# huggingface/parler-tts

Hardware: NVIDIA H100
Metric: audio codec tokens/sec (all codebooks) (higher is better)
Workload: dtype bf16

## Files before the change

### parler_tts_b200/csrc/sample_core.cuh

```cuda
#pragma once
#include "common.cuh"
#include "kernels.h"

namespace ptts {

__device__ __forceinline__ uint32_t fkey(float f) {
  uint32_t u = __float_as_uint(f);
  return (u & 0x80000000u) ? ~u : (u | 0x80000000u);
}

__device__ __forceinline__ void philox_round(uint32_t (&c)[4], uint32_t k0, uint32_t k1) {
  const uint32_t hi0 = __umulhi(0xD2511F53u, c[0]), lo0 = 0xD2511F53u * c[0];
  const uint32_t hi1 = __umulhi(0xCD9E8D57u, c[2]), lo1 = 0xCD9E8D57u * c[2];
  c[0] = hi1 ^ c[1] ^ k0; c[1] = lo1; c[2] = hi0 ^ c[3] ^ k1; c[3] = lo0;
}
__device__ __forceinline__ float philox_uniform(uint64_t seed, uint32_t row, uint32_t col) {
  uint32_t c[4] = {row, col, 0x5054u, 0x5453u};
  uint32_t k0 = (uint32_t)seed, k1 = (uint32_t)(seed >> 32);
#pragma unroll
  for (int i = 0; i < 10; i++) { philox_round(c, k0, k1); k0 += 0x9E3779B9u; k1 += 0xBB67AE85u; }
  return (float)(c[0] >> 8) * (1.0f / 16777216.0f);
}


constexpr int SMP_WARPS = 8;
constexpr int SMP_THREADS = SMP_WARPS * 32;

constexpr int SMP_MAX_ROWS = 3;
struct SmpScratch {
  float f[2][SMP_MAX_ROWS][SMP_WARPS];
  int i[2][SMP_MAX_ROWS][SMP_WARPS];
  int z[2][SMP_MAX_ROWS][SMP_WARPS];
};
__device__ __forceinline__ SmpScratch& smp_scratch() {
  __shared__ SmpScratch sc;
  return sc;
}
constexpr int SMP_BAN_WORDS = 9 * SMP_THREADS / 32;
__device__ __forceinline__ uint32_t (&smp_bans())[SMP_MAX_ROWS][SMP_BAN_WORDS] {
  __shared__ uint32_t ban[SMP_MAX_ROWS][SMP_BAN_WORDS];
  return ban;
}

template <int ITEMS, int R, bool EXT = false>
__device__ __forceinline__ void sample_rows_cta(const SampleArgs& p, const ptts_gen_params& g, const int64_t* __restrict__ forced,
                                                int row0, int stride, int n_rows, int cur_len, ptts_sampling_ext x = {},
                                                SampleOut o = {}) {
  static_assert(R >= 1 && R <= SMP_MAX_ROWS, "rows per pass");
  SmpScratch& sc = smp_scratch();
  float (&s_f)[2][SMP_MAX_ROWS][SMP_WARPS] = sc.f;
  int (&s_i)[2][SMP_MAX_ROWS][SMP_WARPS] = sc.i;
  int (&s_z)[2][SMP_MAX_ROWS][SMP_WARPS] = sc.z;
  const int tid = threadIdx.x, lane = tid & 31, warp = tid >> 5;
  int buf = 0;
  auto cta_sum_i = [&](int (&v)[R]) {
#pragma unroll
    for (int r = 0; r < R; r++) {
      const int w = __reduce_add_sync(0xffffffffu, v[r]);
      if (lane == 0) s_i[buf][r][warp] = w;
    }
    __syncthreads();
#pragma unroll
    for (int r = 0; r < R; r++) {
      int a = 0;
#pragma unroll
      for (int w = 0; w < SMP_WARPS; w++) a += s_i[buf][r][w];
      v[r] = a;
    }
    buf ^= 1;
  };
  auto cta_sum_f = [&](float (&v)[R]) {
#pragma unroll
    for (int r = 0; r < R; r++) {
      const float w = warp_sum(v[r]);
      if (lane == 0) s_f[buf][r][warp] = w;
    }
    __syncthreads();
#pragma unroll
    for (int r = 0; r < R; r++) {
      float a = 0.f;
#pragma unroll
      for (int w = 0; w < SMP_WARPS; w++) a += s_f[buf][r][w];
      v[r] = a;
    }
    buf ^= 1;
  };
  auto cta_max_f = [&](float (&v)[R]) {
#pragma unroll
    for (int r = 0; r < R; r++) {
      const float w = warp_max(v[r]);
      if (lane == 0) s_f[buf][r][warp] = w;
    }
    __syncthreads();
#pragma unroll
    for (int r = 0; r < R; r++) {
      float a = s_f[buf][r][0];
#pragma unroll
      for (int w = 1; w < SMP_WARPS; w++) a = fmaxf(a, s_f[buf][r][w]);
      v[r] = a;
    }
    buf ^= 1;
  };

  int row[R];
  bool valid[R];
  float v[R][ITEMS];
#pragma unroll
  for (int r = 0; r < R; r++) {
    row[r] = row0 + r * stride;
    valid[r] = row[r] < n_rows;
#pragma unroll
    for (int j = 0; j < ITEMS; j++) {
      const int i = tid + SMP_THREADS * j;
      v[r][j] = (valid[r] && i < p.V) ? __ldcg(p.logits + (size_t)row[r] * p.V + i) : -INFINITY;
    }
  }
  auto out_row = [&](float* base, int r) -> float* {
    const int step = cur_len - (g.input_len > 1 ? g.input_len : 1);
    if (base == nullptr || !valid[r] || step < o.first_step || step - o.first_step >= o.n_steps) return nullptr;
    return base + (int64_t)(step - o.first_step) * o.step_stride + (int64_t)row[r] * p.V;
  };
  if constexpr (EXT) {
#pragma unroll
    for (int r = 0; r < R; r++) {
      if (float* dst = out_row(o.logits, r)) {
#pragma unroll
        for (int j = 0; j < ITEMS; j++) {
          const int i = tid + SMP_THREADS * j;
          if (i < p.V) __stcs(dst + i, v[r][j]);
        }
      }
    }
  }
  int t_unf = 0, t_es = 0;
  if (tid < R && row0 + tid * stride < n_rows) { t_unf = p.unfinished[row0 + tid * stride]; t_es = p.eos_seen[row0 + tid * stride]; }
  const int ngram = EXT ? x.no_repeat_ngram_size : 0;
  const bool bans = EXT && ngram > 0 && cur_len + 1 >= ngram;
  if constexpr (EXT) {
    if (bans) {
      uint32_t (&ban)[SMP_MAX_ROWS][SMP_BAN_WORDS] = smp_bans();
#pragma unroll
      for (int r = 0; r < R; r++)
        for (int w = tid; w < SMP_BAN_WORDS; w += SMP_THREADS) ban[r][w] = 0u;
      __syncthreads();
#pragma unroll
      for (int r = 0; r < R; r++) {
        if (!valid[r]) continue;
        const int64_t* h = p.raw_ids + (size_t)row[r] * p.raw_ld;
        const int64_t* tail = h + cur_len - ngram + 1;
        for (int i = tid; i <= cur_len - ngram; i += SMP_THREADS) {
          bool match = true;
          for (int q = 0; q < ngram - 1 && match; q++) match = h[i + q] == tail[q];
          const int64_t t = h[i + ngram - 1];
          if (match && t >= 0 && t < p.V) atomicOr(&ban[r][t >> 5], 1u << (t & 31));
        }
      }
      __syncthreads();
    }
  }
#pragma unroll
  for (int r = 0; r < R; r++) {
    const int b = row[r] / p.K, k = row[r] - b * p.K;
    bool mask_eos = false;
    if (cur_len - (g.input_len > 1 ? g.input_len : 1) < g.min_new_tokens) mask_eos = true;
    if (valid[r]) {
      const int par = cur_len & 1;
      int fu = p.first_unf[par * p.B + b];
      const int es = __ldcg(p.eos_seen + fu);
      if (es > 0 && es <= cur_len && fu < b * p.K + p.K - 1) fu++;
      if (k == 0 && tid == 0) p.first_unf[(par ^ 1) * p.B + b] = fu;
      if (row[r] > fu) mask_eos = true;
    }
#pragma unroll
    for (int j = 0; j < ITEMS; j++) {
      const int i = tid + SMP_THREADS * j;
      if (mask_eos && i == p.eos) v[r][j] = -INFINITY;
      if (g.suppress_special && i >= g.codebook_size) v[r][j] = -INFINITY;
      if constexpr (EXT)
        if (bans && ((smp_bans()[r][i >> 5] >> (i & 31)) & 1u)) v[r][j] = -INFINITY;
    }
  }
  int tok[R];
#pragma unroll
  for (int r = 0; r < R; r++) tok[r] = 0;
  if (g.do_sample) {
    if (g.temperature != 1.0f) {
#pragma unroll
      for (int r = 0; r < R; r++)
#pragma unroll
        for (int j = 0; j < ITEMS; j++) v[r][j] = v[r][j] / g.temperature;
    }
    if (g.top_k > 0) {
      const int kk = g.top_k < p.V ? g.top_k : p.V;
      uint32_t key[R][ITEMS];
      uint32_t th[R];
#pragma unroll
      for (int r = 0; r < R; r++) {
        th[r] = 0;
#pragma unroll
        for (int j = 0; j < ITEMS; j++) key[r][j] = (tid + SMP_THREADS * j < p.V) ? fkey(v[r][j]) : 0u;
      }
      for (int bit = 31; bit >= 0; bit--) {
        int cnt[R];
#pragma unroll
        for (int r = 0; r < R; r++) {
          const uint32_t cand = th[r] | (1u << bit);
          cnt[r] = 0;
#pragma unroll
          for (int j = 0; j < ITEMS; j++) cnt[r] += (key[r][j] >= cand) ? 1 : 0;
        }
        cta_sum_i(cnt);
#pragma unroll
        for (int r = 0; r < R; r++)
          if (cnt[r] >= kk) th[r] |= (1u << bit);
      }
#pragma unroll
      for (int r = 0; r < R; r++)
#pragma unroll
        for (int j = 0; j < ITEMS; j++)
          if (fkey(v[r][j]) < th[r]) v[r][j] = -INFINITY;
    }
    float m[R];
#pragma unroll
    for (int r = 0; r < R; r++) {
      m[r] = -INFINITY;
#pragma unroll
      for (int j = 0; j < ITEMS; j++) m[r] = fmaxf(m[r], v[r][j]);
    }
    cta_max_f(m);
    float e[R][ITEMS];
    float s[R];
#pragma unroll
    for (int r = 0; r < R; r++) {
      s[r] = 0.f;
#pragma unroll
      for (int j = 0; j < ITEMS; j++) { e[r][j] = expf(v[r][j] - m[r]); s[r] += e[r][j]; }
    }
    cta_sum_f(s);
    if (g.top_p < 1.0f) {
      uint32_t th[R];
#pragma unroll
      for (int r = 0; r < R; r++) th[r] = 0;
      for (int bit = 31; bit >= 0; bit--) {
        float c[R];
#pragma unroll
        for (int r = 0; r < R; r++) {
          const uint32_t cand = th[r] | (1u << bit);
          c[r] = 0.f;
#pragma unroll
          for (int j = 0; j < ITEMS; j++) c[r] += (fkey(v[r][j]) <= cand) ? e[r][j] : 0.f;
        }
        cta_sum_f(c);
#pragma unroll
        for (int r = 0; r < R; r++)
          if (c[r] <= (1.0f - g.top_p) * s[r]) th[r] |= (1u << bit);
      }
#pragma unroll
      for (int r = 0; r < R; r++) {
        const uint32_t kmax = fkey(m[r]);
        s[r] = 0.f;
#pragma unroll
        for (int j = 0; j < ITEMS; j++) {
          const uint32_t key = fkey(v[r][j]);
          if (key <= th[r] && key != kmax) { v[r][j] = -INFINITY; e[r][j] = 0.f; }
          s[r] += e[r][j];
        }
      }
      cta_sum_f(s);
    }
    if constexpr (EXT) {
      auto drop_where = [&](auto&& remove) {
#pragma unroll
        for (int r = 0; r < R; r++) {
          const float inv = 1.0f / s[r];
          s[r] = 0.f;
#pragma unroll
          for (int j = 0; j < ITEMS; j++) {
            if (remove(r, j, inv)) { v[r][j] = -INFINITY; e[r][j] = 0.f; }
            s[r] += e[r][j];
          }
        }
        cta_sum_f(s);
      };
      auto entropy = [&](float (&ent)[R], float (&lse)[R]) {
#pragma unroll
        for (int r = 0; r < R; r++) {
          lse[r] = m[r] + logf(s[r]);
          ent[r] = 0.f;
#pragma unroll
          for (int j = 0; j < ITEMS; j++)
            if (v[r][j] > -INFINITY) { const float lp = v[r][j] - lse[r]; ent[r] += lp * expf(lp); }
        }
        cta_sum_f(ent);
#pragma unroll
        for (int r = 0; r < R; r++) ent[r] = -ent[r];
      };
      if (x.min_p > 0.f)
        drop_where([&](int r, int j, float inv) { return e[r][j] * inv < x.min_p * inv; });
      if (x.typical_p < 1.0f) {
        float ent[R], lse[R];
        entropy(ent, lse);
        uint32_t key[R][ITEMS], th[R];
#pragma unroll
        for (int r = 0; r < R; r++) {
          th[r] = 0;
#pragma unroll
          for (int j = 0; j < ITEMS; j++) key[r][j] = fkey(v[r][j] > -INFINITY ? fabsf(lse[r] - v[r][j] - ent[r]) : INFINITY);
        }
        for (int bit = 31; bit >= 0; bit--) {
          float c[R];
#pragma unroll
          for (int r = 0; r < R; r++) {
            const uint32_t cand = th[r] | (1u << bit);
            c[r] = 0.f;
#pragma unroll
            for (int j = 0; j < ITEMS; j++) c[r] += (key[r][j] <= cand) ? e[r][j] : 0.f;
          }
          cta_sum_f(c);
#pragma unroll
          for (int r = 0; r < R; r++)
            if (c[r] < x.typical_p * s[r]) th[r] |= (1u << bit);
        }
        drop_where([&](int r, int j, float) { return th[r] != 0xffffffffu && key[r][j] > th[r] + 1u; });
      }
      if (x.epsilon_cutoff > 0.f)
        drop_where([&](int r, int j, float inv) { return e[r][j] * inv < x.epsilon_cutoff && v[r][j] < m[r]; });
      if (x.eta_cutoff > 0.f) {
        float ent[R], lse[R];
        entropy(ent, lse);
        drop_where([&](int r, int j, float inv) {
          return e[r][j] * inv < fminf(x.eta_cutoff, sqrtf(x.eta_cutoff) * expf(-ent[r])) && v[r][j] < m[r];
        });
      }
    }
    float target[R], carry[R];
    int found[R], last_nz[R];
#pragma unroll
    for (int r = 0; r < R; r++) {
      target[r] = philox_uniform(g.seed, (uint32_t)(row[r] + g.row_base), (uint32_t)cur_len) * s[r];
      carry[r] = 0.f; found[r] = -1; last_nz[r] = -1;
    }
#pragma unroll
    for (int j = 0; j < ITEMS; j++) {
      float x[R];
#pragma unroll
      for (int r = 0; r < R; r++) {
        x[r] = e[r][j];
#pragma unroll
        for (int o = 1; o < 32; o <<= 1) {
          const float y = __shfl_up_sync(0xffffffffu, x[r], o);
          if (lane >= o) x[r] += y;
        }
        if (lane == 31) s_f[buf][r][warp] = x[r];
      }
      __syncthreads();
      float tot[R];
#pragma unroll
      for (int r = 0; r < R; r++) {
        float base = carry[r];
        tot[r] = carry[r];
#pragma unroll
        for (int w = 0; w < SMP_WARPS; w++) {
          const float tw = s_f[buf][r][w];
          if (w < warp) base += tw;
          tot[r] += tw;
        }
        const float cum = base + x[r];
        const unsigned hit = __ballot_sync(0xffffffffu, cum > target[r] && e[r][j] > 0.f);
        const unsigned nz = __ballot_sync(0xffffffffu, e[r][j] > 0.f);
        if (lane == 0) {
          s_i[buf][r][warp] = hit ? SMP_THREADS * j + 32 * warp + (__ffs(hit) - 1) : 0x7fffffff;
          s_z[buf][r][warp] = nz ? SMP_THREADS * j + 32 * warp + (31 - __clz(nz)) : -1;
        }
      }
      __syncthreads();
#pragma unroll
      for (int r = 0; r < R; r++) {
        int first = 0x7fffffff, lastz = -1;
#pragma unroll
        for (int w = 0; w < SMP_WARPS; w++) { first = min(first, s_i[buf][r][w]); lastz = max(lastz, s_z[buf][r][w]); }
        if (found[r] < 0 && first != 0x7fffffff) found[r] = first;
        if (lastz >= 0) last_nz[r] = lastz;
        carry[r] = tot[r];
      }
      buf ^= 1;
    }
#pragma unroll
    for (int r = 0; r < R; r++) tok[r] = found[r] >= 0 ? found[r] : last_nz[r];
    if constexpr (EXT) {
#pragma unroll
      for (int r = 0; r < R; r++)
        if (tok[r] < 0) tok[r] = 0;
    }
  } else {
#pragma unroll
    for (int r = 0; r < R; r++) {
      float m = -INFINITY;
      int mi = 0x7fffffff;
#pragma unroll
      for (int j = 0; j < ITEMS; j++) {
        const int i = tid + SMP_THREADS * j;
        if (i < p.V && (v[r][j] > m || (v[r][j] == m && i < mi))) { m = v[r][j]; mi = i; }
      }
#pragma unroll
      for (int o = 16; o > 0; o >>= 1) {
        const float om = __shfl_xor_sync(0xffffffffu, m, o);
        const int oi = __shfl_xor_sync(0xffffffffu, mi, o);
        if (om > m || (om == m && oi < mi)) { m = om; mi = oi; }
      }
      if (lane == 0) { s_f[buf][r][warp] = m; s_i[buf][r][warp] = mi; }
    }
    __syncthreads();
#pragma unroll
    for (int r = 0; r < R; r++) {
      float m = s_f[buf][r][0];
      int mi = s_i[buf][r][0];
#pragma unroll
      for (int w = 1; w < SMP_WARPS; w++) {
        const float om = s_f[buf][r][w];
        const int oi = s_i[buf][r][w];
        if (om > m || (om == m && oi < mi)) { m = om; mi = oi; }
      }
      tok[r] = mi;
    }
    buf ^= 1;
  }
#pragma unroll
  for (int r = 0; r < R; r++) {
    if (!valid[r]) continue;
#pragma unroll
    for (int j = 0; j < ITEMS; j++) {
      const int i = tid + SMP_THREADS * j;
      if (i < p.V) p.scores[(size_t)row[r] * p.V + i] = v[r][j];
    }
    if constexpr (EXT) {
      if (float* dst = out_row(o.scores, r)) {
#pragma unroll
        for (int j = 0; j < ITEMS; j++) {
          const int i = tid + SMP_THREADS * j;
          if (i < p.V) __stcs(dst + i, v[r][j]);
        }
      }
    }
  }
  int my_tok = 0, my_row = 0;
  bool my_valid = false;
#pragma unroll
  for (int r = 0; r < R; r++)
    if (tid == r) { my_tok = tok[r]; my_row = row[r]; my_valid = valid[r]; }
  if (tid < R && my_valid) {
    const int b = my_row / p.K, k = my_row - b * p.K;
    int t = my_tok;
    if (forced != nullptr) t = (int)forced[my_row];
    if (!t_unf) t = p.pad;
    p.raw_ids[(size_t)my_row * p.raw_ld + cur_len] = t;
    if (t == p.eos && t_es == 0) p.eos_seen[my_row] = cur_len + 1;
    const int new_len = cur_len + 1;
    const int done = (t == p.eos) || (new_len >= g.max_length);
    const int still_unfinished = t_unf && !done;
    p.unfinished[my_row] = still_unfinished;
    int nxt = t;
    if (g.max_length >= 2 * p.K - 1) {
      const bool is_bos = cur_len <= k;
      const bool is_pad = (cur_len - k) >= (g.max_length - p.K + 1);
      if (is_bos || is_pad) nxt = (is_bos ? p.bos : 0) + (is_pad ? p.pad : 0);
      else if (g.input_len > 1 && cur_len - g.input_len < k) nxt = (int)p.prefix_cells[(size_t)my_row * (p.K - 1) + (cur_len - g.input_len)];
    }
    p.cur_ids[my_row] = nxt;
    if (still_unfinished) atomicAdd(&p.ctrl->n_unfinished, 1);
  }
  __syncthreads();
}

template <int ITEMS>
__device__ __forceinline__ void sample_row_cta(const SampleArgs& p, const ptts_gen_params& g, const int64_t* __restrict__ forced,
                                               int row, int cur_len) {
  sample_rows_cta<ITEMS, 1>(p, g, forced, row, 0, row + 1, cur_len);
}

template <int ITEMS>
__device__ __forceinline__ void sample_all_rows_cta(const SampleArgs& p, const ptts_gen_params& g, int cta, int n_ctas, int n_rows, int cur_len) {
  if (n_rows <= n_ctas) {
    if (cta < n_rows) sample_rows_cta<ITEMS, 1>(p, g, nullptr, cta, n_ctas, n_rows, cur_len);
  } else {
    for (int row0 = cta; row0 < n_rows; row0 += 3 * n_ctas) sample_rows_cta<ITEMS, 3>(p, g, nullptr, row0, n_ctas, n_rows, cur_len);
  }
}

}
```

### parler_tts_b200/csrc/step2.cu

```cuda
#include "attn_core.cuh"
#include "common.cuh"
#include "kernels.h"
#include "ln_stats.cuh"
#include "sample_core.cuh"
#include "ptx.cuh"
#include "step.h"
#include "step_common.cuh"
#include <type_traits>

namespace ptts {
namespace cl {

constexpr int C = 2;
constexpr int V = 8;
constexpr int THREADS = 256;
constexpr int ROWS = 32;
constexpr int HROWS = 8;
constexpr int ATT_SMEM = attn_decode_smem_per_warp<bf16>();
constexpr int PROF_STRIDE = 16;
constexpr int QMAX = 6;
constexpr int OFF_STATS = 256, OFF_PART = 512, OFF_RES = 2560, OFF_CVEC = 3584;
constexpr int HDR = 5632;
constexpr int WB_BYTES = 65536;
constexpr int R_OFF = HDR + 2 * WB_BYTES;
// ... 121 lines not shown
  const int dgrp = warp & 1, e4 = warp >> 1;

  uint64_t* abar = reinterpret_cast<uint64_t*>(smem);
  uint64_t* wbar = abar + 1;
  uint64_t* xbar = abar + 3;
  uint64_t* attbars = reinterpret_cast<uint64_t*>(smem + 128);
  float* stats = reinterpret_cast<float*>(smem + OFF_STATS);
  float* part = reinterpret_cast<float*>(smem + OFF_PART);
  float* res_s = reinterpret_cast<float*>(smem + OFF_RES);
  float* cvec = reinterpret_cast<float*>(smem + OFF_CVEC);
  unsigned char* Rg = smem + R_OFF;
  const uint32_t peer_xbar = mapa(smem_u32(xbar), (uint32_t)peer);
  uint32_t par_a = 0, par_w = 0, par_x = 0, att_parity = 0;

  if (tid == 0) {
    mbar_init<1>(abar); mbar_init<1>(&wbar[0]); mbar_init<1>(&wbar[1]); mbar_init<1>(xbar);
    asm volatile("fence.mbarrier_init.release.cluster;" ::: "memory");
  }
  attention_decode_init_warp(attbars + 2 * warp, lane);
  cluster_arrive(); cluster_wait();
  unsigned* const bar_ctr = p.bar + (gen & 1u);
  unsigned bar_target = 0u;
  if (cta == 0 && tid == 0) p.bar[(gen + 1u) & 1u] = 0u;

  const char* blob = p.blob;
  long long* const prof0 = (p.prof != nullptr && cta == 0) ? p.prof : nullptr;
  long long* prof = prof0;
  prof_mark(prof, 0);

  auto issue_weight_job = [&](int j) {
    const char* src; uint32_t bytes;
    if (!weight_job(p, j, cta, rank, src, bytes)) return;
    mbar_expect_tx(&wbar[j & 1], bytes);
    bulk_g2s_evict_first(smem + HDR + (j & 1) * WB_BYTES, src, bytes, &wbar[j & 1]);
  };
  __shared__ int s_next_active;
  const int n_steps = (p.do_sample_phase && p.n_steps > 1 && prof0 == nullptr) ? p.n_steps : 1;
  int unfinished_prev = 0;
#pragma unroll 1
  for (int it = 0; it < n_steps; it++) {
  pos = p.P + cur_len - 1;
  prof = prof0;
  cluster_arrive_reuse();
  if (tid == 0) { issue_weight_job(0); issue_weight_job(1); }

  bf16* const x_img = p.cl_x;
  bf16* const a_img = p.cl_attn;
  bf16* const h_img = p.cl_h;
  const int x_slice_elems = ROWS * pitch, h_slice_elems = ROWS * pitchF;
  auto h_offset = [&](int n) {
    const int lk = klocal(n >> 5), kq = KsF >> 5;
    return (size_t)(2 * kslice(n >> 5) + lk / kq) * h_slice_elems + (lk % kq) * 32 + (n & 31);
  };
  const int xo_slice = kslice(cta >> 2), xo_col = klocal(cta >> 2) * 32 + (cta & 3) * 8;

  {
    const int row = tid >> 3, f = tid & 7, n = cta * 8 + f;
    const float v = row < B ? embed_value(p, row, n, pos) : 0.f;
    res_s[row * 8 + f] = v;
    x_img[(size_t)xo_slice * x_slice_elems + row * pitch + xo_col + f] = __float2bfloat16_rn(v);
  }
  prof_mark(prof, 6);
  auto request_slice = [&](const bf16* img_slice, uint32_t bytes) {
    fence_proxy_async_smem();
    mbar_expect_tx(abar, bytes);
    bulk_g2s(Rg, img_slice, bytes, abar);
  };
  auto slice_of = [&](int sub, const bf16*& img, uint32_t& bytes) {
    if (sub == PH_QKV || sub == PH_QC) { img = x_img + (size_t)rank * x_slice_elems + (size_t)(HROWS * rblk) * pitch; bytes = (uint32_t)(HROWS * pitch * 2); }
    else if (sub == PH_O || sub == PH_OC) { img = a_img + (size_t)rank * x_slice_elems; bytes = (uint32_t)(x_slice_elems * 2); }
    else if (sub == PH_FC1) { img = x_img + (size_t)rank * x_slice_elems; bytes = (uint32_t)(x_slice_elems * 2); }
    else { img = h_img + (size_t)(2 * rank) * h_slice_elems; bytes = (uint32_t)(h_slice_elems * 2); }
  };
  {
    const bf16* nimg; uint32_t nbytes;
    slice_of(PH_QKV, nimg, nbytes);
    bar_target = grid_sync(bar_ctr, bar_target, -1, false, nullptr, [&]() { request_slice(nimg, nbytes); });
  }
  prof_mark(prof, 7);

  const int lrow = (lane & 7) + ((lane >> 3) & 1) * 8, lcol = (lane >> 4) * 8;
  const int g = lane >> 2, t4 = lane & 3;
  const int n_phases = 6 * p.L;

  const int att_row = HROWS * rblk + 4 * rank + (warp >> 1);
  const int att_slice = kslice(2 * head), att_col = klocal(2 * head) * 32;

#pragma unroll 1
  for (int ph = 0; ph < n_phases; ph++) {
    const int l = ph / 6, sub = ph - 6 * l;
    prof = prof0 ? prof0 + (size_t)(ph + 1) * PROF_STRIDE : nullptr;
    prof_mark(prof, 0);
    const char* lb = blob + p.lay.layer0 + p.lay.layer_stride * l;
    const bool rowpart = (sub == PH_QKV || sub == PH_QC);
    const bool has_ln = (sub == PH_QKV || sub == PH_QC || sub == PH_FC1);
    const int q = (sub == PH_QKV) ? 6 : (sub == PH_QC ? 2 : (sub == PH_FC1 ? qe : 1));
    const int Nc = 4 * q * 8;
    const int KT = (sub == PH_FC2 ? KsF : Ks) >> 5;
    const int apitch = (sub == PH_FC2) ? pitchF : pitch;
    const int act_bytes = (rowpart ? HROWS : ROWS) * apitch * 2;
    const int RS = (q == 1) ? 8 : 8 * q + 2;
    const int blk = rowpart ? 32 + 4 * 16 * q * 4 : 256 + ROWS * RS * 4;
    unsigned char* const recv = Rg + ((act_bytes + 127) & ~127);
    const uint32_t peer_recv = mapa(smem_u32(recv), (uint32_t)peer);
    const uint32_t xbytes = 4u * (rowpart ? V * 4 * 16 * q + V / 2 * 4 * 2 : V / C * (ROWS * 8 * q + (has_ln ? ROWS * 2 : 0)));
    auto put = [&](int d, uint32_t off, auto v) {
      if (d == rank) *reinterpret_cast<decltype(v)*>(recv + off) = v;
      else st_async(peer_recv + off, v, peer_xbar);
    };
    const int j0 = JOBS_PER_LAYER * l + (sub == 0 ? 0 : sub + QKV_JOBS - 1);
    if (tid == 0) mbar_expect_tx(xbar, xbytes);

    auto att_stage0 = [&]() -> unsigned char* {
      if (sub == PH_QC) return Rg + ATT_S0_QC + warp * ATT_STAGE;
      return warp < 6 ? Rg + ATT_S0_QKV + warp * ATT_STAGE : smem + HDR + (warp - 6) * WB_BYTES + ATT_S0_WB;
    };
    if (rowpart && att_row < B)
      attention_decode_request<bf16>(decode_attn_args(p, l, pos, sub == PH_QC), att_row, head, pos, att_stage0(), attbars + 2 * warp, lane, warp & 1, 2);

    float cv1 = 0.f, cv2 = 0.f;
    if (has_ln) {
      const float* c1; int ntot;
      if (sub == PH_QKV) { c1 = reinterpret_cast<const float*>(lb + p.lay.c_qkv); ntot = p.qkv_rows; }
      else if (sub == PH_QC) { c1 = reinterpret_cast<const float*>(lb + p.lay.c_qc); ntot = H; }
      else { c1 = reinterpret_cast<const float*>(lb + p.lay.c_fc1); ntot = F; }
      const int nown = rowpart ? Nc : 8 * q;
      if (tid < nown) {
        int n;
        if (sub == PH_QKV) n = (tid >> 6) * (p.nh * HD) + head * HD + (tid & 63);
        else if (sub == PH_QC) n = head * HD + tid;
        else n = cta * 8 * q + tid;
        cv1 = c1[n];
        cv2 = c1[ntot + n];
      }
    }

    auto wait_job = [&](int j) {
      mbar_wait(&wbar[j & 1], (par_w >> (j & 1)) & 1u, 1);
      par_w ^= 1u << (j & 1);
    };
    auto ring = [&](int j) { return reinterpret_cast<const uint4*>(smem + HDR + (j & 1) * WB_BYTES) + lane; };
    wait_job(j0);
    if (sub == PH_QKV) wait_job(j0 + 1);
    mbar_wait(abar, par_a, 0);
    par_a ^= 1u;
    prof_mark(prof, 1);
    float acc[2][QMAX][4];
    RowStatFrag rst;
    row_stat_zero(rst);
    {
      const bf16* xs = reinterpret_cast<const bf16*>(Rg);
      if (rowpart) {
        auto head_pass = [&](auto pass_tag) {
          constexpr int P = decltype(pass_tag)::value;
          const int u = 2 * P + dgrp;
          float t[2][QMAX][4];
          if (sub == PH_QKV) mma_slice<6, 1, P == 0>(t, rst, xs, apitch, ring(j0 + u), KT, e4, KT, lrow & 7, lcol);
          else mma_slice<2, 1, P == 0>(t, rst, xs, apitch, ring(j0) + (size_t)(2 * u) * KT * 32, KT, e4, KT, lrow & 7, lcol);
          const int d = g >> 2;
          const uint32_t slot = (uint32_t)((8 * rank + warp) * blk);
          if (P == 0) {
            cluster_wait();
            if (dgrp == 0) {
              const uint32_t so = slot + 8 * (g & 3);
              if (t4 == 0) put(d, so, rst.s1[0][0]);
              if (t4 == (g >> 1)) put(d, so + 4, (g & 1) ? rst.sq[0][0][1] : rst.sq[0][0][0]);
// ... 87 lines not shown
      if (row < B && sub == PH_FC1 && q == 4) {
        const int f = 4 * f0;
        float v[4] = {0.f, 0.f, 0.f, 0.f};
#pragma unroll
        for (int sv = 0; sv < V; sv++) {
          const float* bp = reinterpret_cast<const float*>(recv + (size_t)sv * blk + 256) + row * RS + f;
          const float2 a = *reinterpret_cast<const float2*>(bp), b2 = *reinterpret_cast<const float2*>(bp + 2);
          v[0] += a.x; v[1] += a.y; v[2] += b2.x; v[3] += b2.y;
        }
#pragma unroll
        for (int e = 0; e < 4; e++) v[e] = apply_act(DT<bf16>::rnd(ln_rstd * (v[e] - ln_mean * cvec[f + e]) + cvec[256 + f + e]), p.act);
        uint2 pk;
        pk.x = att_pack(v[0], v[1]); pk.y = att_pack(v[2], v[3]);
        *reinterpret_cast<uint2*>(h_img + h_offset(cta * 32 + f) + row * pitchF) = pk;
      } else if (row < B) {
        for (int i = 0; i < q; i++) {
          const int f = f0 + 8 * i;
          float v = 0.f;
#pragma unroll
          for (int sv = 0; sv < V; sv++) v += reinterpret_cast<const float*>(recv + (size_t)sv * blk + 256)[row * RS + f];
          if (sub == PH_FC1) {
            v = ln_rstd * (v - ln_mean * cvec[f]) + cvec[256 + f];
            v = apply_act(DT<bf16>::rnd(v), p.act);
            h_img[h_offset(cta * 8 * q + f) + row * pitchF] = __float2bfloat16_rn(v);
          } else {
            v = DT<bf16>::rnd(res_s[row * 8 + f] + DT<bf16>::rnd(v));
            res_s[row * 8 + f] = v;
            x_img[(size_t)xo_slice * x_slice_elems + row * pitch + xo_col + f] = __float2bfloat16_rn(v);
          }
        }
      }
    } else {
      bf16* qkv_s = reinterpret_cast<bf16*>(Rg + QKV_OFF);
      auto gather = [&](auto jw_tag) {
        constexpr int JW = decltype(jw_tag)::value, NC = 4 * JW, QCW = 2 * JW;
        for (int idx = tid; idx < 4 * NC; idx += THREADS) {
          const int r4 = idx / NC, col = idx - r4 * NC;
          const int u = col / JW, cw = (u >> 1) * JW + (col - u * JW);
          float S1 = 0.f, S2 = 0.f;
#pragma unroll
          for (int e = 0; e < V; e++) {
            const float2 x = *reinterpret_cast<const float2*>(recv + (size_t)(8 * (e >> 2) + 2 * (e & 3)) * blk + r4 * 8);
            S1 += x.x; S2 += x.y;
          }
          const float ln_mean = S1 / (float)H;
          const float ln_rstd = rsqrtf(fmaxf(S2 / (float)H - ln_mean * ln_mean, 0.f) + p.eps);
          float v = 0.f;
#pragma unroll
          for (int e = 0; e < V; e++)
            v += reinterpret_cast<const float*>(recv + (size_t)(8 * (e >> 2) + 2 * (e & 3) + (u & 1)) * blk + 32)[r4 * QCW + cw];
          v = ln_rstd * (v - ln_mean * cvec[col]) + cvec[256 + col];
          qkv_s[idx] = __float2bfloat16_rn(v);
        }
      };
      if (sub == PH_QKV) gather(std::integral_constant<int, 48>{}); else gather(std::integral_constant<int, 16>{});
      static_assert(HD == 64, "QKV: 2 x 2 units of 6 n-tiles (q|k|v of a head), q_cross: 2 x 2 units of 2 n-tiles");
    }
    prof_mark(prof, 4);
    __syncthreads();
    cluster_arrive_reuse();

    if (rowpart) {
      if (att_row < B) {
        AttnArgs att = decode_attn_args(p, l, pos, sub == PH_QC);
        const bf16* qkv_s = reinterpret_cast<const bf16*>(Rg + QKV_OFF);
        const int row_base = HROWS * rblk + 4 * rank;
        const bf16* qbase = qkv_s - (size_t)row_base * Nc - (size_t)head * HD;
        att.q = qbase; att.ldq = Nc;
        att.ldo = pitch;
        att.out = a_img + (size_t)att_slice * x_slice_elems + att_col - (size_t)head * HD;
        if (sub == PH_QKV) { att.knew = qbase; att.vnew = qbase; att.ldkv = Nc; att.k_col0 = HD; att.v_col0 = 2 * HD; }
        unsigned char* wb0 = smem + HDR;
        unsigned char* held = wb0 + ((sub == PH_QKV ? j0 + 1 : j0) & 1) * WB_BYTES;
        unsigned char* other = wb0 + ((sub == PH_QKV ? j0 : j0 + 1) & 1) * WB_BYTES;
        unsigned char* rest = warp < 2 ? Rg + (size_t)warp * ATT_REST : held + (size_t)(warp - 2) * ATT_REST;
        float* xr = reinterpret_cast<float*>(other + 16384) + (warp >> 1) * 128;
        prof_mark(prof, 10);
        attention_decode_sweep<bf16>(att, att_row, head, pos, att_stage0(), rest, attbars + 2 * warp, lane, att_parity, warp & 1, 2, xr, (warp >> 1) + 1,
                                     true, tid == 0 ? prof : nullptr);
      }
      prof_mark(prof, 5);
    }
    prof_mark(prof, 6);
    if (p.prof != nullptr && l == p.L / 2 && tid == 0) {
      unsigned long long ns;
      asm volatile("mov.u64 %0, %%globaltimer;" : "=l"(ns));
      p.prof[(size_t)(n_phases + 4) * PROF_STRIDE + sub * (int)gridDim.x + cta] = (long long)ns;
    }

    const bool last = (ph + 1 == n_phases);
    const bf16* nimg; uint32_t nbytes;
    if (last) { nimg = x_img; nbytes = (uint32_t)(C * x_slice_elems * 2); }
    else slice_of((sub + 1) % 6, nimg, nbytes);
    const int held_job = sub == PH_QKV ? j0 + QKV_JOBS + 1 : (sub == PH_QC || sub == PH_OC) ? j0 + 2 : -1;
    bar_target = grid_sync(bar_ctr, bar_target, ph, false, nullptr, [&]() {
      request_slice(nimg, nbytes);
      if (held_job >= 0) issue_weight_job(held_job);
    });
    prof_mark(prof, 7);
  }
  cluster_wait();

  prof = prof0 ? prof0 + (size_t)(n_phases + 1) * PROF_STRIDE : nullptr;
  prof_mark(prof, 0);
  {
    const int ntasks = p.K * p.V / 32;
    const float* c1 = reinterpret_cast<const float*>(blob + p.lay.c_heads);
    const float* c2 = c1 + p.K * p.V;
    mbar_wait(abar, par_a, 3);
    par_a ^= 1u;
    const bf16* xs = reinterpret_cast<const bf16*>(Rg);
    const int KTH = H >> 5;
    auto ktile = [&](int kt) { return xs + (size_t)kslice(kt) * x_slice_elems + klocal(kt) * 32; };
    {
      RowStatFrag rst;
      row_stat_zero(rst);
      for (int kt = warp; kt < KTH; kt += 8) {
        const bf16* sl = ktile(kt);
#pragma unroll
        for (int mt = 0; mt < 2; mt++)
#pragma unroll
          for (int j = 0; j < 2; j++) {
            uint32_t a[4];
            ldmatrix_x4(a, sl + (size_t)(mt * 16 + lrow) * pitch + j * 16 + lcol);
            row_stat_mma(rst, mt, a);
          }
      }
      row_stat_store(rst, part, warp, lane);
      __syncthreads();
      row_stat_finalize(part, H, ROWS, p.eps, stats);
      __syncthreads();
    }
    prof_mark(prof, 1);
    constexpr int HRS = 40;
    int job = JOBS_PER_LAYER * p.L;
    for (int task = cta; task < ntasks; task += (int)gridDim.x, job++) {
      mbar_wait(&wbar[job & 1], (par_w >> (job & 1)) & 1u, 4);
      par_w ^= 1u << (job & 1);
      float acc[2][4][4];
#pragma unroll
      for (int a = 0; a < 2; a++)
#pragma unroll
        for (int j = 0; j < 4; j++)
#pragma unroll
          for (int e = 0; e < 4; e++) acc[a][j][e] = 0.f;
      unsigned char* wbuf = smem + HDR + (job & 1) * WB_BYTES;
      const uint4* wb = reinterpret_cast<const uint4*>(wbuf) + lane;
      for (int kt = warp; kt < KTH; kt += 8) {
        const bf16* sl = ktile(kt);
        uint32_t a[2][2][4];
#pragma unroll
        for (int mt = 0; mt < 2; mt++)
#pragma unroll
          for (int j = 0; j < 2; j++) ldmatrix_x4(a[mt][j], sl + (size_t)(mt * 16 + lrow) * pitch + j * 16 + lcol);
#pragma unroll
        for (int j = 0; j < 4; j++) {
          const uint4 w = wb[((size_t)j * KTH + kt) * 32];
#pragma unroll
          for (int mt = 0; mt < 2; mt++) {
            mma_bf16_16816(acc[mt][j], a[mt][0], w.x, w.y);
            mma_bf16_16816(acc[mt][j], a[mt][1], w.z, w.w);
          }
        }
      }
      __syncthreads();
      float* red = reinterpret_cast<float*>(wbuf);
#pragma unroll
      for (int mt = 0; mt < 2; mt++)
#pragma unroll
        for (int j = 0; j < 4; j++) {
          float* base = red + ((size_t)warp * 32 + mt * 16 + g) * HRS + j * 8 + 2 * t4;
          *reinterpret_cast<float2*>(base) = make_float2(acc[mt][j][0], acc[mt][j][1]);
          *reinterpret_cast<float2*>(base + 8 * HRS) = make_float2(acc[mt][j][2], acc[mt][j][3]);
        }
      __syncthreads();
      {
        const int er = tid >> 3, ec = tid & 7;
        if (er < B) {
          const float mean = stats[2 * er], rstd = stats[2 * er + 1];
#pragma unroll
          for (int j = 0; j < 4; j++) {
            const int cidx = j * 8 + ec, n = task * 32 + cidx;
            float v = 0.f;
#pragma unroll
            for (int w = 0; w < 8; w++) v += red[((size_t)w * 32 + er) * HRS + cidx];
            p.logits[(size_t)er * p.K * p.V + n] = DT<bf16>::rnd(rstd * (v - mean * c1[n]) + c2[n]);
          }
        }
      }
      __syncthreads();
      if (tid == 32) {
        fence_proxy_async_smem();
        issue_weight_job(job + 2);
      }
    }
  }
  prof_mark(prof, 6);
  bar_target = grid_sync(bar_ctr, bar_target, n_phases, true);
  prof = prof0 ? prof0 + (size_t)(n_phases + 2) * PROF_STRIDE : nullptr;
  prof_mark(prof, 0);
  if (p.do_sample_phase) {
    const ptts_gen_params gp = *p.sa.gen;
    const int BK = B * p.K;
    sample_phase<ITEMS>(p.sa, gp, BK, cur_len);
    prof_mark(prof, 1);
    bar_target = grid_sync(bar_ctr, bar_target, n_phases + 1, true, nullptr, [&]() {
      const int tot = *reinterpret_cast<volatile int*>(&ctrl->n_unfinished);
      s_next_active = (tot - unfinished_prev > 0) ? 1 : 0;
      unfinished_prev = tot;
    });
    prof_mark(prof, 2);
  }
  bool go_on = false;
  if (p.do_sample_phase) {
    const int act = s_next_active;
    if (cta == 0 && tid == 0) {
      ctrl->cur_len = cur_len + 1;
      ctrl->active = act;
      ctrl->steps_run += 1;
    }
    go_on = act != 0;
    cur_len += 1;
  }
  if (!go_on) break;
  }
  if (cta == 0 && tid == 0) {
    if (p.do_sample_phase) ctrl->n_unfinished = 0;
    ctrl->launch_gen = (int)(gen + 1u);
  }
}

__global__ void cluster_pack_kernel(const uint4* __restrict__ src, uint4* __restrict__ dst, int ph, int nh, int ntc, int kts, int KT_src) {
  const int64_t tile = blockIdx.x;
  const int ktl = (int)(tile % kts);
  const int j = (int)((tile / kts) % ntc);
  const int slice = (int)(tile / ((int64_t)kts * ntc));
  const int rank = slice & 1, owner = slice >> 1;
  int n_tile;
  if (ph == PH_QKV) n_tile = (j >> 3) * (nh * 8) + owner * 8 + (j & 7);
  else n_tile = owner * ntc + j;
  const int kt = kglobal(rank, ktl);
  dst[tile * 32 + threadIdx.x] = src[((int64_t)n_tile * KT_src + kt) * 32 + threadIdx.x];
}

}

int cluster_pack_layer(const DecoderLayout& L, char* layer, cudaStream_t st) {
  for (int ph = 0; ph < 6; ph++) {
    const ClusterPhase cp = cluster_phase(L, ph);
    const int64_t tiles = (int64_t)cp.owners * cl::C * cp.nt * cp.kt;
    cl::cluster_pack_kernel<<<(unsigned)tiles, 32, 0, st>>>(reinterpret_cast<const uint4*>(layer + cp.mat),
                                                            reinterpret_cast<uint4*>(layer + L.cp[ph]), ph, L.nh, cp.nt, cp.kt, cp.kt_src);
  }
  PTTS_LAUNCH_CHECK();
  return PTTS_OK;
}

static const void* cluster_kernel_fn(const StepParams& p) {
  if (p.sample_items <= 1) return (const void*)cl::decode_step_cluster_kernel<1>;
  if (p.sample_items <= 5) return (const void*)cl::decode_step_cluster_kernel<5>;
  return (const void*)cl::decode_step_cluster_kernel<9>;
}

static void cluster_launch_config(const StepParams& p, cudaLaunchConfig_t& cfg, cudaLaunchAttribute* at, cudaStream_t st) {
  cfg = cudaLaunchConfig_t{};
  cfg.gridDim = dim3((unsigned)(4 * p.nh * cl::C));
  cfg.blockDim = dim3(cl::THREADS);
  cfg.dynamicSmemBytes = cl::SMEM_BYTES;
  cfg.stream = st;
  at[0].id = cudaLaunchAttributeClusterDimension;
  at[0].val.clusterDim.x = cl::C; at[0].val.clusterDim.y = 1; at[0].val.clusterDim.z = 1;
  at[1].id = cudaLaunchAttributeCooperative;
  at[1].val.cooperative = 1;
  cfg.attrs = at;
  cfg.numAttrs = 2;
}

bool cluster_step_available(const StepParams& p) {
  const void* fn = cluster_kernel_fn(p);
  static bool told = false;
  auto why = [&](const char* what, cudaError_t e, int n) {
    if (!told) fprintf(stderr, "ptts_b200: cluster step kernel not used (%s: %s, %d co-resident clusters of %d, need %d); the one-CTA-per-SM step kernel runs instead\n",
                       what, cudaGetErrorString(e), n, cl::C, 4 * p.nh);
    told = true;
    cudaGetLastError();
    return false;
  };
  cudaError_t e = cudaFuncSetAttribute(fn, cudaFuncAttributeMaxDynamicSharedMemorySize, cl::SMEM_BYTES);
// ... 22 lines not shown
```

### parler_tts_b200/csrc/step_common.cuh

```cuda
#pragma once
#include "attn_core.cuh"
#include "common.cuh"
#include "sample_core.cuh"
#include "step.h"

namespace ptts {

__device__ __forceinline__ float embed_value(const StepParams& p, int row, int col, int pos) {
  const bf16* tables = reinterpret_cast<const bf16*>(p.blob + p.lay.embed);
  float v = 0.f;
#pragma unroll 1
  for (int k0 = 0; k0 < p.K; k0 += 8) {
    float ev[8];
#pragma unroll
    for (int k = 0; k < 8; k++)
      if (k0 + k < p.K) ev[k] = __bfloat162float(tables[((size_t)(k0 + k) * (p.V + 1) + p.sa.cur_ids[row * p.K + k0 + k]) * p.H + col]);
#pragma unroll
    for (int k = 0; k < 8; k++)
      if (k0 + k < p.K) v = (k0 + k == 0) ? ev[k] : DT<bf16>::rnd(v + ev[k]);
  }
  if (!p.rope) v = DT<bf16>::rnd(v + __bfloat162float(reinterpret_cast<const bf16*>(p.blob + p.lay.pos)[(size_t)pos * p.H + col]));
  return v;
}

__device__ __forceinline__ AttnArgs decode_attn_args(const StepParams& p, int l, int pos, bool cross) {
  AttnArgs a{};
  a.ctrl = nullptr; a.B = p.B; a.nh = p.nh; a.q_len = 1;
  a.past_from_ctrl = 0; a.past_len = pos; a.prefix = p.P;
  a.rope = p.rope; a.rope_cos = p.blob + p.lay.rope_cos; a.rope_sin = p.blob + p.lay.rope_sin; a.scale = p.scale;
  if (!cross) {
    char* kc = p.self_kv + p.self_layer_stride * l;
    a.kcache = kc; a.vcache = kc + (size_t)p.B * p.nkv * p.Tmax * HD * 2;
    a.kv_b_stride = (int64_t)p.nkv * p.Tmax * HD; a.kv_h_stride = (int64_t)p.Tmax * HD; a.kv_t_stride = HD; a.kv_b_div = 1;
    a.key_mask = p.prompt_mask; a.mask_len = p.P; a.mask_ld = p.P;
    a.nkv = p.nkv; a.cross = 0; a.kv_len = 0; a.kv_capacity = p.Tmax;
  } else {
    char* ck = p.cross_kv + p.cross_layer_stride * l;
    a.kcache = ck; a.vcache = ck + (size_t)(p.B / p.takes) * p.nckv * p.S * HD * 2;
    a.kv_b_stride = (int64_t)p.nckv * p.S * HD; a.kv_h_stride = (int64_t)p.S * HD; a.kv_t_stride = HD; a.kv_b_div = p.takes;
    a.key_mask = p.enc_mask; a.mask_len = p.S; a.mask_ld = p.S;
    a.nkv = p.nckv; a.cross = 1; a.kv_len = p.S; a.kv_capacity = p.S;
  }
  return a;
}

template <int ITEMS>
__device__ __noinline__ void sample_phase(const SampleArgs& sa, const ptts_gen_params& gp, int BK, int cur_len) {
  sample_all_rows_cta<ITEMS>(sa, gp, (int)blockIdx.x, (int)gridDim.x, BK, cur_len);
}

}
```

Baseline: 256,100.

## Use radix-histogram top-k selection and a single-barrier multinomial scan in sampling

Top-k threshold search moves from a 32-step bitwise binary search (one CTA-wide reduction and barrier per bit) to a 4-pass 8-bit radix select using shared-memory histograms built with match_any plus atomics. The multinomial inverse-CDF scan now stores per-warp totals for all item slots at once, so it needs two barriers in total instead of two per slot. This cuts block-wide synchronisations in the per-step sampling phase, at the cost of shared-memory atomics and extra shared memory. Profiling timestamps are also added, gated on a profiling pointer.

New measurement: 259,300, median of 6. 1.01x the previous value.

```diff
diff --git a/parler_tts_b200/csrc/sample_core.cuh b/parler_tts_b200/csrc/sample_core.cuh
--- a/parler_tts_b200/csrc/sample_core.cuh
+++ b/parler_tts_b200/csrc/sample_core.cuh
@@ -1,6 +1,7 @@
 #pragma once
 #include "common.cuh"
 #include "kernels.h"
+#include "ptx.cuh"
 
 namespace ptts {
 
@@ -36,6 +37,15 @@
   __shared__ SmpScratch sc;
   return sc;
 }
+constexpr int SMP_MAX_ITEMS = 9;
+union SmpWide {
+  uint32_t hist[SMP_MAX_ROWS][128];
+  float tot[SMP_MAX_ROWS][SMP_MAX_ITEMS][SMP_WARPS];
+};
+__device__ __forceinline__ SmpWide& smp_wide() {
+  __shared__ SmpWide w;
+  return w;
+}
 constexpr int SMP_BAN_WORDS = 9 * SMP_THREADS / 32;
 __device__ __forceinline__ uint32_t (&smp_bans())[SMP_MAX_ROWS][SMP_BAN_WORDS] {
   __shared__ uint32_t ban[SMP_MAX_ROWS][SMP_BAN_WORDS];
@@ -45,30 +55,14 @@
 template <int ITEMS, int R, bool EXT = false>
 __device__ __forceinline__ void sample_rows_cta(const SampleArgs& p, const ptts_gen_params& g, const int64_t* __restrict__ forced,
                                                 int row0, int stride, int n_rows, int cur_len, ptts_sampling_ext x = {},
-                                                SampleOut o = {}) {
-  static_assert(R >= 1 && R <= SMP_MAX_ROWS, "rows per pass");
+                                                SampleOut o = {}, long long* prof = nullptr) {
+  static_assert(R >= 1 && R <= SMP_MAX_ROWS && ITEMS <= SMP_MAX_ITEMS, "rows per pass, slots per thread");
   SmpScratch& sc = smp_scratch();
   float (&s_f)[2][SMP_MAX_ROWS][SMP_WARPS] = sc.f;
   int (&s_i)[2][SMP_MAX_ROWS][SMP_WARPS] = sc.i;
   int (&s_z)[2][SMP_MAX_ROWS][SMP_WARPS] = sc.z;
   const int tid = threadIdx.x, lane = tid & 31, warp = tid >> 5;
   int buf = 0;
-  auto cta_sum_i = [&](int (&v)[R]) {
-#pragma unroll
-    for (int r = 0; r < R; r++) {
-      const int w = __reduce_add_sync(0xffffffffu, v[r]);
-      if (lane == 0) s_i[buf][r][warp] = w;
-    }
-    __syncthreads();
-#pragma unroll
-    for (int r = 0; r < R; r++) {
-      int a = 0;
-#pragma unroll
-      for (int w = 0; w < SMP_WARPS; w++) a += s_i[buf][r][w];
-      v[r] = a;
-    }
-    buf ^= 1;
-  };
   auto cta_sum_f = [&](float (&v)[R]) {
 #pragma unroll
     for (int r = 0; r < R; r++) {
@@ -180,6 +174,7 @@
         if (bans && ((smp_bans()[r][i >> 5] >> (i & 31)) & 1u)) v[r][j] = -INFINITY;
     }
   }
+  prof_mark(prof, 4);
   int tok[R];
 #pragma unroll
   for (int r = 0; r < R; r++) tok[r] = 0;
@@ -200,19 +195,62 @@
 #pragma unroll
         for (int j = 0; j < ITEMS; j++) key[r][j] = (tid + SMP_THREADS * j < p.V) ? fkey(v[r][j]) : 0u;
       }
-      for (int bit = 31; bit >= 0; bit--) {
-        int cnt[R];
+      uint32_t (&hist)[SMP_MAX_ROWS][128] = smp_wide().hist;
+      int above[R];
+#pragma unroll
+      for (int r = 0; r < R; r++) {
+        above[r] = 0;
+        if (tid < 128) hist[r][tid] = 0u;
+      }
+      __syncthreads();
+#pragma unroll 1
+      for (int pass = 0; pass < 4; pass++) {
+        const int shift = 24 - 8 * pass;
+        const uint32_t hi = pass == 0 ? 0u : 0xffffffffu << (shift + 8);
+#pragma unroll
+        for (int r = 0; r < R; r++)
+#pragma unroll
+          for (int j = 0; j < ITEMS; j++) {
+            const bool in = tid + SMP_THREADS * j < p.V && ((key[r][j] ^ th[r]) & hi) == 0u;
+            const uint32_t d = in ? (key[r][j] >> shift) & 255u : 256u;
+            const unsigned same = __match_any_sync(0xffffffffu, d);
+            if (in && lane == __ffs(same) - 1) atomicAdd(&hist[r][d >> 1], (uint32_t)__popc(same) << (16 * (d & 1u)));
+          }
+        __syncthreads();
+        if (warp < R) {
+          int ab = 0;
+#pragma unroll
+          for (int r = 0; r < R; r++)
+            if (r == warp) ab = above[r];
+          int c[8], ls = 0;
+#pragma unroll
+          for (int q = 0; q < 4; q++) {
+            const uint32_t w = hist[warp][4 * lane + q];
+            hist[warp][4 * lane + q] = 0u;
+            c[2 * q] = (int)(w & 0xffffu);
+            c[2 * q + 1] = (int)(w >> 16);
+            ls += c[2 * q] + c[2 * q + 1];
+          }
+          int suf = ls;
+#pragma unroll
+          for (int o = 1; o < 32; o <<= 1) {
+            const int y = __shfl_down_sync(0xffffffffu, suf, o);
+            if (lane + o < 32) suf += y;
+          }
+          int run = ab + suf - ls;
+#pragma unroll
+          for (int b = 7; b >= 0; b--) {
+            if (run < kk && run + c[b] >= kk) { s_i[buf][warp][0] = 8 * lane + b; s_i[buf][warp][1] = run; }
+            run += c[b];
+          }
+        }
+        __syncthreads();
 #pragma unroll
         for (int r = 0; r < R; r++) {
-          const uint32_t cand = th[r] | (1u << bit);
-          cnt[r] = 0;
-#pragma unroll
-          for (int j = 0; j < ITEMS; j++) cnt[r] += (key[r][j] >= cand) ? 1 : 0;
-        }
-        cta_sum_i(cnt);
-#pragma unroll
-        for (int r = 0; r < R; r++)
-          if (cnt[r] >= kk) th[r] |= (1u << bit);
+          th[r] |= (uint32_t)s_i[buf][r][0] << shift;
+          above[r] = s_i[buf][r][1];
+        }
+        buf ^= 1;
       }
 #pragma unroll
       for (int r = 0; r < R; r++)
@@ -220,6 +258,7 @@
         for (int j = 0; j < ITEMS; j++)
           if (fkey(v[r][j]) < th[r]) v[r][j] = -INFINITY;
     }
+    prof_mark(prof, 5);
     float m[R];
 #pragma unroll
     for (int r = 0; r < R; r++) {
@@ -333,60 +372,55 @@
         });
       }
     }
-    float target[R], carry[R];
-    int found[R], last_nz[R];
-#pragma unroll
-    for (int r = 0; r < R; r++) {
-      target[r] = philox_uniform(g.seed, (uint32_t)(row[r] + g.row_base), (uint32_t)cur_len) * s[r];
-      carry[r] = 0.f; found[r] = -1; last_nz[r] = -1;
-    }
-#pragma unroll
-    for (int j = 0; j < ITEMS; j++) {
-      float x[R];
-#pragma unroll
-      for (int r = 0; r < R; r++) {
-        x[r] = e[r][j];
+    prof_mark(prof, 6);
+    float (&wtot)[SMP_MAX_ROWS][SMP_MAX_ITEMS][SMP_WARPS] = smp_wide().tot;
+    float xs[R][ITEMS];
+#pragma unroll
+    for (int r = 0; r < R; r++)
+#pragma unroll
+      for (int j = 0; j < ITEMS; j++) {
+        float x = e[r][j];
 #pragma unroll
         for (int o = 1; o < 32; o <<= 1) {
-          const float y = __shfl_up_sync(0xffffffffu, x[r], o);
-          if (lane >= o) x[r] += y;
-        }
-        if (lane == 31) s_f[buf][r][warp] = x[r];
-      }
-      __syncthreads();
-      float tot[R];
-#pragma unroll
-      for (int r = 0; r < R; r++) {
-        float base = carry[r];
-        tot[r] = carry[r];
+          const float y = __shfl_up_sync(0xffffffffu, x, o);
+          if (lane >= o) x += y;
+        }
+        xs[r][j] = x;
+        if (lane == 31) wtot[r][j][warp] = x;
+      }
+    __syncthreads();
+#pragma unroll
+    for (int r = 0; r < R; r++) {
+      const float target = philox_uniform(g.seed, (uint32_t)(row[r] + g.row_base), (uint32_t)cur_len) * s[r];
+      float carry = 0.f;
+      int first = 0x7fffffff, lastz = -1;
+#pragma unroll
+      for (int j = 0; j < ITEMS; j++) {
+        float base = carry, tot = carry;
 #pragma unroll
         for (int w = 0; w < SMP_WARPS; w++) {
-          const float tw = s_f[buf][r][w];
+          const float tw = wtot[r][j][w];
           if (w < warp) base += tw;
-          tot[r] += tw;
-        }
-        const float cum = base + x[r];
-        const unsigned hit = __ballot_sync(0xffffffffu, cum > target[r] && e[r][j] > 0.f);
+          tot += tw;
+        }
+        const float cum = base + xs[r][j];
+        const unsigned hit = __ballot_sync(0xffffffffu, cum > target && e[r][j] > 0.f);
         const unsigned nz = __ballot_sync(0xffffffffu, e[r][j] > 0.f);
-        if (lane == 0) {
-          s_i[buf][r][warp] = hit ? SMP_THREADS * j + 32 * warp + (__ffs(hit) - 1) : 0x7fffffff;
-          s_z[buf][r][warp] = nz ? SMP_THREADS * j + 32 * warp + (31 - __clz(nz)) : -1;
-        }
-      }
-      __syncthreads();
-#pragma unroll
-      for (int r = 0; r < R; r++) {
-        int first = 0x7fffffff, lastz = -1;
-#pragma unroll
-        for (int w = 0; w < SMP_WARPS; w++) { first = min(first, s_i[buf][r][w]); lastz = max(lastz, s_z[buf][r][w]); }
-        if (found[r] < 0 && first != 0x7fffffff) found[r] = first;
-        if (lastz >= 0) last_nz[r] = lastz;
-        carry[r] = tot[r];
-      }
-      buf ^= 1;
-    }
-#pragma unroll
-    for (int r = 0; r < R; r++) tok[r] = found[r] >= 0 ? found[r] : last_nz[r];
+        if (hit && first == 0x7fffffff) first = SMP_THREADS * j + 32 * warp + (__ffs(hit) - 1);
+        if (nz) lastz = SMP_THREADS * j + 32 * warp + (31 - __clz(nz));
+        carry = tot;
+      }
+      if (lane == 0) { s_i[buf][r][warp] = first; s_z[buf][r][warp] = lastz; }
+    }
+    __syncthreads();
+#pragma unroll
+    for (int r = 0; r < R; r++) {
+      int first = 0x7fffffff, lastz = -1;
+#pragma unroll
+      for (int w = 0; w < SMP_WARPS; w++) { first = min(first, s_i[buf][r][w]); lastz = max(lastz, s_z[buf][r][w]); }
+      tok[r] = first != 0x7fffffff ? first : lastz;
+    }
+    buf ^= 1;
     if constexpr (EXT) {
 #pragma unroll
       for (int r = 0; r < R; r++)
@@ -425,6 +459,7 @@
     }
     buf ^= 1;
   }
+  prof_mark(prof, 7);
 #pragma unroll
   for (int r = 0; r < R; r++) {
     if (!valid[r]) continue;
@@ -479,12 +514,13 @@
 }
 
 template <int ITEMS>
-__device__ __forceinline__ void sample_all_rows_cta(const SampleArgs& p, const ptts_gen_params& g, int cta, int n_ctas, int n_rows, int cur_len) {
+__device__ __forceinline__ void sample_all_rows_cta(const SampleArgs& p, const ptts_gen_params& g, int cta, int n_ctas, int n_rows, int cur_len,
+                                                    long long* prof = nullptr) {
   if (n_rows <= n_ctas) {
-    if (cta < n_rows) sample_rows_cta<ITEMS, 1>(p, g, nullptr, cta, n_ctas, n_rows, cur_len);
+    if (cta < n_rows) sample_rows_cta<ITEMS, 1>(p, g, nullptr, cta, n_ctas, n_rows, cur_len, {}, {}, prof);
   } else {
-    for (int row0 = cta; row0 < n_rows; row0 += 3 * n_ctas) sample_rows_cta<ITEMS, 3>(p, g, nullptr, row0, n_ctas, n_rows, cur_len);
-  }
-}
-
-}
+    for (int row0 = cta; row0 < n_rows; row0 += 3 * n_ctas) sample_rows_cta<ITEMS, 3>(p, g, nullptr, row0, n_ctas, n_rows, cur_len, {}, {}, prof);
+  }
+}
+
+}
diff --git a/parler_tts_b200/csrc/step2.cu b/parler_tts_b200/csrc/step2.cu
--- a/parler_tts_b200/csrc/step2.cu
+++ b/parler_tts_b200/csrc/step2.cu
@@ -227,6 +227,12 @@
   const int lrow = (lane & 7) + ((lane >> 3) & 1) * 8, lcol = (lane >> 4) * 8;
   const int g = lane >> 2, t4 = lane & 3;
   const int n_phases = 6 * p.L;
+  auto cta_time = [&](int slot) {
+    if (p.prof == nullptr || tid != 0) return;
+    unsigned long long ns;
+    asm volatile("mov.u64 %0, %%globaltimer;" : "=l"(ns));
+    p.prof[(size_t)(n_phases + 4) * PROF_STRIDE + slot * (int)gridDim.x + cta] = (long long)ns;
+  };
 
   const int att_row = HROWS * rblk + 4 * rank + (warp >> 1);
   const int att_slice = kslice(2 * head), att_col = klocal(2 * head) * 32;
@@ -480,11 +486,7 @@
       prof_mark(prof, 5);
     }
     prof_mark(prof, 6);
-    if (p.prof != nullptr && l == p.L / 2 && tid == 0) {
-      unsigned long long ns;
-      asm volatile("mov.u64 %0, %%globaltimer;" : "=l"(ns));
-      p.prof[(size_t)(n_phases + 4) * PROF_STRIDE + sub * (int)gridDim.x + cta] = (long long)ns;
-    }
+    if (l == p.L / 2) cta_time(sub);
 
     const bool last = (ph + 1 == n_phases);
     const bf16* nimg; uint32_t nbytes;
@@ -594,14 +596,16 @@
     }
   }
   prof_mark(prof, 6);
+  cta_time(6);
   bar_target = grid_sync(bar_ctr, bar_target, n_phases, true);
   prof = prof0 ? prof0 + (size_t)(n_phases + 2) * PROF_STRIDE : nullptr;
   prof_mark(prof, 0);
   if (p.do_sample_phase) {
     const ptts_gen_params gp = *p.sa.gen;
     const int BK = B * p.K;
-    sample_phase<ITEMS>(p.sa, gp, BK, cur_len);
+    sample_phase<ITEMS>(p.sa, gp, BK, cur_len, prof);
     prof_mark(prof, 1);
+    cta_time(7);
     bar_target = grid_sync(bar_ctr, bar_target, n_phases + 1, true, nullptr, [&]() {
       const int tot = *reinterpret_cast<volatile int*>(&ctrl->n_unfinished);
       s_next_active = (tot - unfinished_prev > 0) ? 1 : 0;
diff --git a/parler_tts_b200/csrc/step_common.cuh b/parler_tts_b200/csrc/step_common.cuh
--- a/parler_tts_b200/csrc/step_common.cuh
+++ b/parler_tts_b200/csrc/step_common.cuh
@@ -45,8 +45,8 @@
 }
 
 template <int ITEMS>
-__device__ __noinline__ void sample_phase(const SampleArgs& sa, const ptts_gen_params& gp, int BK, int cur_len) {
-  sample_all_rows_cta<ITEMS>(sa, gp, (int)blockIdx.x, (int)gridDim.x, BK, cur_len);
+__device__ __noinline__ void sample_phase(const SampleArgs& sa, const ptts_gen_params& gp, int BK, int cur_len, long long* prof = nullptr) {
+  sample_all_rows_cta<ITEMS>(sa, gp, (int)blockIdx.x, (int)gridDim.x, BK, cur_len, prof);
 }
 
 }
```
